# omid-arhami/topolow

Measured on AMD Instinct MI355X. Metric: relaxation iterations/sec (NxN pairs), higher is better.
Workload: dtype f32

## Files before the change

topolow_amd/csrc/relax_symm.h:

```cpp
#pragma once

#include <hip/hip_runtime.h>
#include <algorithm>
#include <type_traits>
#include <vector>
#include "relax_common.h"

namespace topolow {

#ifndef TOPOLOW_SYM_MINW
#define TOPOLOW_SYM_MINW 2
#endif
constexpr int kSymRows = 64;
constexpr int kSymCols = 32;
constexpr int kSymTileWords = kSymRows * kSymCols;
constexpr int kSymWaves = 4;

template <int DIM> struct SymRec { static constexpr int W = (DIM + 2 + 3) & ~3; };

struct SymUnit {
  int tile_row;
  int j0, j1;
  int tile0;
};

TL_HD inline long long sym_tile_index(int R, int J, int TC) { return (long long)R * TC - (long long)R * (R - 1) + (J - 2 * R); }
TL_HD inline size_t sym_word_in_tile(int r, int c) {
  const int a = r >> 3, p = (r & 7) >> 1, e = r & 1, b = c >> 2, h = (c & 3) >> 1, f = c & 1;
  return (size_t)((((4 * h + p) * 64) + a + 8 * b) * 4 + 2 * (f ^ (a & 1)) + e);
}

struct alignas(32) SymRun {
  int u0, u1;
  SymUnit first;
  int tiles;
  int reserved;
};
struct SymPlan {
  std::vector<SymUnit> units;
  std::vector<int> wave_first;
  std::vector<int2> row_units;
  std::vector<SymRun> runs() const {
    std::vector<SymRun> r(wave_first.size() - 1);
    for (size_t w = 0; w + 1 < wave_first.size(); ++w) {
      r[w].u0 = wave_first[w];
      r[w].u1 = wave_first[w + 1];
      r[w].first = r[w].u0 < r[w].u1 ? units[r[w].u0] : SymUnit{0, 0, 0, 0};
      r[w].tiles = 0;
      for (int u = r[w].u0; u < r[w].u1; ++u) r[w].tiles += units[u].j1 - units[u].j0;
      r[w].reserved = 0;
    }
    return r;
  }
};
inline SymPlan relax_symm_plan(int npad, int n_waves, long long t0 = 0, long long t1 = -1, int* r_first = nullptr,
                               int* r_last = nullptr) {
  SymPlan P;
  const int TR = npad / kSymRows, TC = npad / kSymCols;
  if (t1 < 0) t1 = (long long)TR * (TR + 1);
  const long long total = t1 - t0;
  int rf = -1, rl = -1;
  for (int R = 0; R < TR; ++R) {
    const long long a = sym_tile_index(R, 2 * R, TC), b = a + (TC - 2 * R);
// ... 63 lines not shown
  for (int R = 0; R < TR; ++R) {
    int j0 = 0, j1 = 0;
    rows_j(R, j0, j1);
    if (j1 > j0) total += j1 - j0;
  }
  P.wave_first.assign(n_waves + 1, 0);
  P.row_units.assign(TR, int2{0, 0});
  if (total == 0) return P;
  long long done = 0;
  int w = 0;
  long long w_end = (total * (w + 1) + n_waves - 1) / n_waves;
  for (int R = 0; R < TR; ++R) {
    P.row_units[R].x = (int)P.units.size();
    int j = 0, j_end = 0;
    rows_j(R, j, j_end);
    while (j < j_end) {
      while (done >= w_end && w + 1 < n_waves) {
        ++w;
        P.wave_first[w] = (int)P.units.size();
        w_end = (total * (w + 1) + n_waves - 1) / n_waves;
      }
      const int take = (int)std::min<long long>(j_end - j, std::max<long long>(w_end - done, 1));
      P.units.push_back({R, j, j + take, (int)sym_tile_index(R, j, TC)});
      j += take;
      done += take;
    }
    P.row_units[R].y = (int)P.units.size() - P.row_units[R].x;
  }
  for (int q = w + 1; q <= n_waves; ++q) P.wave_first[q] = (int)P.units.size();
  return P;
}

typedef float symf2 __attribute__((ext_vector_type(2)));
#ifdef TOPOLOW_SYM_STAMPS
__device__ unsigned long long* g_sym_stamps = nullptr;
#endif

#define TL_SYM_DPP_ADD(v, ctrl) asm volatile("v_add_f32_dpp %0, %0, %0 " ctrl " row_mask:0xf bank_mask:0xf" : "+v"(v))
template <int NV>
__device__ __forceinline__ void sym_col_reduce(float (&first)[NV], float (&second)[NV]) {
#pragma unroll
  for (int q = 0; q < NV; ++q) asm volatile("" : "+v"(first[q]), "+v"(second[q]));
  asm volatile("s_nop 1");
#pragma unroll
  for (int q = 0; q < NV; ++q)
    asm volatile("v_add_f32_dpp %0, %1, %0 quad_perm:[1,0,3,2] row_mask:0xf bank_mask:0xf" : "+v"(first[q]) : "v"(second[q]));
  if constexpr (NV < 3) asm volatile("s_nop 1");
#pragma unroll
  for (int q = 0; q < NV; ++q) TL_SYM_DPP_ADD(first[q], "quad_perm:[2,3,0,1]");
  if constexpr (NV < 3) asm volatile("s_nop 1");
#pragma unroll
  for (int q = 0; q < NV; ++q) TL_SYM_DPP_ADD(first[q], "row_shl:4");
}

template <int DIM, bool THR, bool ERR, bool CNT, bool FIRST>
__device__ __forceinline__ void sym_pair(const float (&pc)[DIM], float ksc, float cgc, const symf2 (&pi2)[DIM],
                                         symf2 ks2, symf2 cg2, uint32_t w0, uint32_t w1, symf2 (&racc2)[DIM],
                                         symf2 (&cacc2)[DIM], symf2& err2, unsigned& cnt_wave ) {
  symf2 dx[DIM];
  symf2 s = {0.0f, 0.0f};
#pragma unroll
  for (int d = 0; d < DIM; ++d) {
    const symf2 pcd = {pc[d], pc[d]};
    dx[d] = pcd - pi2[d];
    s = __builtin_elementwise_fma(dx[d], dx[d], s);
  }
  const symf2 r = {__builtin_amdgcn_sqrtf(s.x), __builtin_amdgcn_sqrtf(s.y)};
  const symf2 rs = r + (symf2){0.01f, 0.01f};
  const symf2 inv = {__builtin_amdgcn_rcpf(rs.x), __builtin_amdgcn_rcpf(rs.y)};
  const symf2 t = {bits_f32(THR ? (w0 & ~kCodeMask) : w0), bits_f32(THR ? (w1 & ~kCodeMask) : w1)};
  bool sp0, sp1;
  if constexpr (THR) {
    const symf2 e0 = t - r;
    auto decide = [](uint32_t w, float e) {
      const uint32_t flip = (w << 30) & 0x80000000u;
      const int32_t some = (int32_t)(((w >> 1) | w) << 31) >> 31;
      const uint32_t q = ((f32_bits(e) ^ flip) & (uint32_t)some) | (0x3f800000u & ~(uint32_t)some);
      return bits_f32(q) > 0.0f;
    };
    sp0 = decide(w0, e0.x);
    sp1 = decide(w1, e0.y);
  } else {
    sp0 = __builtin_amdgcn_classf(bits_f32(w0), 0x1f8);
    sp1 = __builtin_amdgcn_classf(bits_f32(w1), 0x1f8);
  }
  const symf2 e = t - r;
  const symf2 inv2 = inv * inv;
  const symf2 u = {sp0 ? e.x : inv2.x, sp1 ? e.y : inv2.y};
  const symf2 base = u * inv;
  const symf2 mr = {sp0 ? ks2.x : cg2.x, sp1 ? ks2.y : cg2.y};
  const symf2 coef = base * mr;
#pragma unroll
  for (int d = 0; d < DIM; ++d) racc2[d] = __builtin_elementwise_fma(dx[d], coef, racc2[d]);
  const symf2 mc = {sp0 ? ksc : cgc, sp1 ? ksc : cgc};
  const symf2 cc = base * mc;
#pragma unroll
  for (int d = 0; d < DIM; ++d)
    cacc2[d] = FIRST ? dx[d] * cc : __builtin_elementwise_fma(dx[d], cc, cacc2[d]);
  if constexpr (ERR) {
    const symf2 a = {sp0 ? fabsf(e.x) : 0.0f, sp1 ? fabsf(e.y) : 0.0f};
    err2 += a;
    if constexpr (CNT) cnt_wave += (sp0 ? 1u : 0u) + (sp1 ? 1u : 0u);
  }
}

template <int DIM, bool ANYTHR, bool ERR>
__global__ __launch_bounds__(64 * kSymWaves, TOPOLOW_SYM_MINW) void symm_sweep_kernel(
    const uint32_t* __restrict__ enc, const float* __restrict__ rec, const SymUnit* __restrict__ units,
    const SymRun* __restrict__ runs, float* __restrict__ rowpart, float* __restrict__ colpart, int npad,
    const RunState* st, double* __restrict__ part_sum, unsigned long long* __restrict__ part_cnt,
    unsigned long long fixed_cnt, int col_row0, int prio) {
  const int wave = __builtin_amdgcn_readfirstlane(threadIdx.x >> 6);
  const int gw = blockIdx.x * kSymWaves + wave;
  const SymRun run = runs[gw];
  int stopped = st->stopped;
  if constexpr (ERR)
    asm("" : "+s"(stopped) : "s"(run.u0), "s"(run.u1), "s"(run.first.tile_row), "s"(run.first.j0), "s"(run.first.j1),
        "s"(run.first.tile0), "s"(run.tiles), "s"(enc), "s"(rec), "s"(units),
        "s"(rowpart), "s"(colpart), "s"(npad), "s"(col_row0), "s"(prio), "s"(part_sum), "s"(part_cnt), "s"(fixed_cnt));
  else
    asm("" : "+s"(stopped) : "s"(run.u0), "s"(run.u1), "s"(run.first.tile_row), "s"(run.first.j0), "s"(run.first.j1),
        "s"(run.first.tile0), "s"(run.tiles), "s"(enc), "s"(rec), "s"(units),
        "s"(rowpart), "s"(colpart), "s"(npad), "s"(col_row0), "s"(prio));
  if (stopped) return;
#ifdef TOPOLOW_SYM_STAMPS
  const unsigned long long stamp_c0 = __builtin_amdgcn_s_memtime(), stamp_r0 = __builtin_amdgcn_s_memrealtime();
#endif
  constexpr int W = SymRec<DIM>::W;
  constexpr int kRecVec = W / 4;
  constexpr int kTileVec = kSymCols * kRecVec;
  constexpr int kLdsVec = kTileVec + kSymCols / 4;
  __shared__ uint4 lds[kSymWaves][2][kLdsVec];
  auto lds_slot = [](int q) { return q + (q / (4 * kRecVec)); };
  const int lane = threadIdx.x & 63;
  const int a = lane & 7, b = lane >> 3;

  const int u_begin = __builtin_amdgcn_readfirstlane(run.u0);
  const int u_end = __builtin_amdgcn_readfirstlane(run.u1);
  typedef unsigned int u32x4 __attribute__((ext_vector_type(4)));
  const __amdgpu_buffer_rsrc_t rec_rsrc = __builtin_amdgcn_make_buffer_rsrc(const_cast<float*>(rec), 0, npad * W * 4, 0x00020000);
  int left = __builtin_amdgcn_readfirstlane(run.tiles);
  const int lv3 = (3 * left) >> 2, lv2 = left >> 1, lv1 = left >> 2;
  SymUnit U_next = run.first;
  for (int u = u_begin; u < u_end; ++u) {
    const SymUnit U = U_next;
    U_next = units[u + 1 < u_end ? u + 1 : u];
    const int R = __builtin_amdgcn_readfirstlane(U.tile_row);
    const int J0 = __builtin_amdgcn_readfirstlane(U.j0), J1 = __builtin_amdgcn_readfirstlane(U.j1);
    __builtin_assume(J0 < J1);
    const int slot = u;
    const int tile0 = __builtin_amdgcn_readfirstlane(U.tile0);

    symf2 pi2[4][DIM], ks2[4], cg2[4], racc2[4][DIM];
    {
      const uint4* rr = reinterpret_cast<const uint4*>(rec + (size_t)(R * kSymRows + 8 * a) * W);
#pragma unroll
      for (int p = 0; p < 4; ++p) {
        float f[2][W];
#pragma unroll
        for (int e = 0; e < 2; ++e)
#pragma unroll
          for (int v = 0; v < kRecVec; ++v) {
            const uint4 q = rr[(2 * p + e) * kRecVec + v];
            f[e][4 * v + 0] = __builtin_bit_cast(float, q.x);
            f[e][4 * v + 1] = __builtin_bit_cast(float, q.y);
            f[e][4 * v + 2] = __builtin_bit_cast(float, q.z);
            f[e][4 * v + 3] = __builtin_bit_cast(float, q.w);
          }
#pragma unroll
        for (int d = 0; d < DIM; ++d) {
          pi2[p][d] = (symf2){f[0][d], f[1][d]};
          racc2[p][d] = (symf2){0.0f, 0.0f};
        }
        ks2[p] = (symf2){f[0][DIM], f[1][DIM]};
        cg2[p] = (symf2){f[0][DIM + 1], f[1][DIM + 1]};
      }
    }
    const __amdgpu_buffer_rsrc_t rsrc = __builtin_amdgcn_make_buffer_rsrc(
        const_cast<uint32_t*>(enc) + (size_t)tile0 * kSymTileWords, 0, (J1 - J0) * kSymTileWords * 4, 0x00020000);
    const __amdgpu_buffer_rsrc_t col_rsrc = __builtin_amdgcn_make_buffer_rsrc(colpart + (size_t)(R - col_row0) * npad * DIM, 0, npad * DIM * 4, 0x00020000);
    const int col_off = a < 2 ? (4 * b + a) * DIM * 4 : 0x40000000;
    const int swap = a & 1;
    auto request = [&](int J, int h, u32x4 (&dst)[4]) {
#pragma unroll
      for (int p = 0; p < 4; ++p)
        dst[p] = __builtin_amdgcn_raw_buffer_load_b128(rsrc, lane * 16 + ((J - J0) * 8 + 4 * h + p) * 1024, 0, 0);
    };
    u32x4 wa[4], wb[4];
    request(J0, 0, wa);
    const uint4* recv = reinterpret_cast<const uint4*>(rec);
    if (lane < kTileVec) lds[wave][J0 & 1][lds_slot(lane)] = recv[(size_t)J0 * kTileVec + lane];
    if constexpr (kTileVec > 64) if (lane + 64 < kTileVec) lds[wave][J0 & 1][lds_slot(lane + 64)] = recv[(size_t)J0 * kTileVec + lane + 64];

    symf2 err2 = {0.0f, 0.0f};
    float err_unit = 0.0f;
    unsigned cnt_wave = 0, cnt_unit2 = 0;
    auto read_rec = [&](int J, int idx, float (&f)[W]) {
      const int col = idx ^ swap;
      const uint4* cp = &lds[wave][J & 1][4 * b * kRecVec + b];
#pragma unroll
      for (int v = 0; v < kRecVec; ++v) {
        const uint4 q = cp[col * kRecVec + v];
        f[4 * v + 0] = __builtin_bit_cast(float, q.x);
        f[4 * v + 1] = __builtin_bit_cast(float, q.y);
        f[4 * v + 2] = __builtin_bit_cast(float, q.z);
        f[4 * v + 3] = __builtin_bit_cast(float, q.w);
      }
    };
    float f_first[W];
    read_rec(J0, 0, f_first);
#pragma unroll 1
    for (int J = J0; J < J1; ++J) {
      if (prio) {
        if (left > lv3) __builtin_amdgcn_s_setprio(3);
        else if (left > lv2) __builtin_amdgcn_s_setprio(2);
        else if (left > lv1) __builtin_amdgcn_s_setprio(1);
        else __builtin_amdgcn_s_setprio(0);
      }
      --left;
      const int Jn = J + 1 < J1 ? J + 1 : J;
      request(J, 1, wb);
      u32x4 rn0 = {0, 0, 0, 0}, rn1 = {0, 0, 0, 0};
      rn0 = __builtin_amdgcn_raw_buffer_load_b128(rec_rsrc, (Jn * kTileVec + lane) * 16, 0, 0);
      if constexpr (kTileVec > 64) rn1 = __builtin_amdgcn_raw_buffer_load_b128(rec_rsrc, (Jn * kTileVec + lane + 64) * 16, 0, 0);
      __builtin_amdgcn_sched_barrier(0);

      const bool diag = J < 2 * R + 2;
      float fq[4][W];
#pragma unroll
      for (int q = 0; q < W; ++q) fq[0][q] = f_first[q];
      auto half = [&](auto hc, const u32x4 (&wc)[4]) {
        constexpr int h = decltype(hc)::value;
        symf2 cacc2[2][DIM];
#pragma unroll
        for (int c = 0; c < 2; ++c) {
          if (2 * h + c + 1 < 4) {
            read_rec(J, 2 * h + c + 1, fq[2 * h + c + 1]);
            __builtin_amdgcn_sched_barrier(0);
          }
          const float (&f)[W] = fq[2 * h + c];
          float pc[DIM];
#pragma unroll
          for (int d = 0; d < DIM; ++d) pc[d] = f[d];
          const float ksc = f[DIM], cgc = f[DIM + 1];
#pragma unroll
          for (int p = 0; p < 4; ++p) {
            const uint32_t w0 = c == 0 ? wc[p].x : wc[p].z, w1 = c == 0 ? wc[p].y : wc[p].w;
            if (p == 0)
              sym_pair<DIM, ANYTHR, ERR, ANYTHR, true>(pc, ksc, cgc, pi2[p], ks2[p], cg2[p], w0, w1, racc2[p], cacc2[c], err2, cnt_wave);
            else
              sym_pair<DIM, ANYTHR, ERR, ANYTHR, false>(pc, ksc, cgc, pi2[p], ks2[p], cg2[p], w0, w1, racc2[p], cacc2[c], err2, cnt_wave);
          }
        }
        float first[DIM], second[DIM];
#pragma unroll
        for (int d = 0; d < DIM; ++d) {
          first[d] = cacc2[0][d].x + cacc2[0][d].y;
          second[d] = cacc2[1][d].x + cacc2[1][d].y;
        }
        sym_col_reduce<DIM>(first, second);
        const int off0 = col_off + ((J * kSymCols) * DIM + h * 2 * DIM) * 4;
#pragma unroll
        for (int q = 0; q < DIM; q += 4) {
          if (q + 4 <= DIM) {
            const u32x4 pk = {__builtin_bit_cast(uint32_t, first[q]), __builtin_bit_cast(uint32_t, first[q + 1]),
                              __builtin_bit_cast(uint32_t, first[q + 2]), __builtin_bit_cast(uint32_t, first[q + 3])};
            __builtin_amdgcn_raw_buffer_store_b128(pk, col_rsrc, off0 + q * 4, 0, 0);
          } else {
#pragma unroll
            for (int t = q; t < DIM; ++t)
              __builtin_amdgcn_raw_buffer_store_b32(__builtin_bit_cast(uint32_t, first[t]), col_rsrc, off0 + t * 4, 0, 0);
          }
        }
      };
      half(std::integral_constant<int, 0>{}, wa);
      request(Jn, 0, wa);
      __builtin_amdgcn_sched_barrier(0);
      half(std::integral_constant<int, 1>{}, wb);
      if constexpr (ERR) {
        const float es = err2.x + err2.y;
        err_unit += diag ? es : 2.0f * es;
        cnt_unit2 += diag ? cnt_wave : 2u * cnt_wave;
        err2 = (symf2){0.0f, 0.0f};
        cnt_wave = 0;
      }
      __builtin_amdgcn_sched_barrier(0);
      if (lane < kTileVec) lds[wave][(J + 1) & 1][lds_slot(lane)] = make_uint4(rn0.x, rn0.y, rn0.z, rn0.w);
      if constexpr (kTileVec > 64) if (lane + 64 < kTileVec) lds[wave][(J + 1) & 1][lds_slot(lane + 64)] = make_uint4(rn1.x, rn1.y, rn1.z, rn1.w);
      read_rec(J + 1, 0, f_first);
    }
#pragma unroll
    for (int p = 0; p < 4; ++p)
#pragma unroll
      for (int d = 0; d < DIM; ++d) {
        symf2 v = racc2[p][d];
        v.x += __shfl_xor(v.x, 8, 64);  v.y += __shfl_xor(v.y, 8, 64);
        v.x += __shfl_xor(v.x, 16, 64); v.y += __shfl_xor(v.y, 16, 64);
        v.x += __shfl_xor(v.x, 32, 64); v.y += __shfl_xor(v.y, 32, 64);
        racc2[p][d] = v;
      }
    if (b == 0) {
      float* dst = rowpart + ((size_t)slot * kSymRows + 8 * a) * DIM;
#pragma unroll
      for (int p = 0; p < 4; ++p)
#pragma unroll
        for (int d = 0; d < DIM; ++d) {
          dst[(2 * p) * DIM + d] = racc2[p][d].x;
          dst[(2 * p + 1) * DIM + d] = racc2[p][d].y;
        }
    }
    if constexpr (ERR) {
      double s = (double)err_unit;
#pragma unroll
      for (int m = 32; m >= 1; m >>= 1) s += __shfl_xor(s, m, 64);
      if constexpr (ANYTHR) {
#pragma unroll
        for (int m = 32; m >= 1; m >>= 1) cnt_unit2 += __shfl_xor(cnt_unit2, m, 64);
      }
      if (lane == 0) {
        part_sum[slot] = s;
        part_cnt[slot] = ANYTHR ? (unsigned long long)cnt_unit2 : (slot == 0 ? fixed_cnt : 0ull);
      }
    }
  }
#ifdef TOPOLOW_SYM_STAMPS
  if (lane == 0 && g_sym_stamps != nullptr) {
    g_sym_stamps[4 * gw] = __builtin_amdgcn_s_memtime() - stamp_c0;
    g_sym_stamps[4 * gw + 1] = stamp_r0;
    g_sym_stamps[4 * gw + 2] = __builtin_amdgcn_s_memrealtime();
    unsigned hw_id, xcc_id;
    asm volatile("s_getreg_b32 %0, hwreg(HW_REG_HW_ID)" : "=s"(hw_id));
    asm volatile("s_getreg_b32 %0, hwreg(HW_REG_XCC_ID)" : "=s"(xcc_id));
    g_sym_stamps[4 * gw + 3] = ((unsigned long long)xcc_id << 32) | hw_id;
  }
#endif
}

template <int DIM, typename real> struct SymReal;
template <int DIM> struct SymReal<DIM, float> {
  static constexpr int W = SymRec<DIM>::W;
  __device__ static float ks(double k, float g) { return (float)(2.0 * k) / (4.0f * g + (float)k); }
  __device__ static float cg(double c_rep, float g) { return (float)(0.5 * c_rep) / g; }
  __device__ static float far(int) { return kFarF32; }
};

#ifndef TL_APPLY_PARTS
#define TL_APPLY_PARTS 16
#endif
constexpr int kSymApplyParts = TL_APPLY_PARTS;
template <int DIM, typename real>
__global__ __launch_bounds__(32 * kSymApplyParts) void symm_apply_kernel(
    const real* __restrict__ rec, real* __restrict__ rec_next, real* __restrict__ pos_out, const float* __restrict__ gplus,
    const real* __restrict__ rowpart, const real* __restrict__ colpart, const int2* __restrict__ row_units, int n,
    int npad, double k_next, double c_rep, int iter1, RunState* st, int rr_stages = 0, int rr_stage = 0) {
// ... 81 lines not shown
}

__global__ __launch_bounds__(256) void symm_tiles_kernel(const uint32_t* const* __restrict__ src, const int* __restrict__ row0,
                                                        int n_src, int ld, uint32_t* __restrict__ tenc, int TC,
                                                        long long t_first) {
  const long long t = t_first + blockIdx.x;
  int R = 0;
  {
    const double b = (double)TC + 1.0;
    const double disc = b * b - 4.0 * (double)t;
    R = (int)((b - sqrt(disc > 0.0 ? disc : 0.0)) * 0.5);
    while (R > 0 && (long long)R * TC - (long long)R * (R - 1) > t) --R;
    while ((long long)(R + 1) * TC - (long long)(R + 1) * R <= t) ++R;
  }
  const int J = 2 * R + (int)(t - ((long long)R * TC - (long long)R * (R - 1)));
  uint32_t* dst = tenc + (size_t)blockIdx.x * kSymTileWords;
  const int rows = row0[n_src];
#pragma unroll
  for (int q = 0; q < kSymTileWords / 256; ++q) {
    const int cell = threadIdx.x + q * 256;
    const int r = cell >> 5, c = cell & 31;
    const int row = R * kSymRows + r, col = J * kSymCols + c;
    uint32_t w = kInfWord;
    if (row < rows && col < ld) {
      int blk = 0;
      while (blk + 1 < n_src && row >= row0[blk + 1]) ++blk;
      w = src[blk][enc_index(row - row0[blk], col, ld)];
    }
    const int a = r >> 3, p = (r & 7) >> 1, e = r & 1, b = c >> 2, h = (c & 3) >> 1, f = c & 1;
    dst[(((4 * h + p) * 64) + a + 8 * b) * 4 + 2 * (f ^ (a & 1)) + e] = w;
  }
}


template <int DIM>
__global__ __launch_bounds__(32 * 32) void symm_partial_kernel(
    const float* __restrict__ rowpart, const float* __restrict__ colpart, const int2* __restrict__ row_units, int r_first,
    int r_last, int n, int npad, float* const* __restrict__ inbox, const int* __restrict__ own0, int n_own, int slot,
    const RunState* st) {
  if (st != nullptr && st->stopped) return;
  __shared__ float red[32][kSymCols][DIM];
  const int R = blockIdx.x >> 1;
  const int part = threadIdx.x >> 5, pt = threadIdx.x & 31;
  const int i = blockIdx.x * kSymCols + pt;
  float acc[DIM];
#pragma unroll
  for (int d = 0; d < DIM; ++d) acc[d] = 0.0f;
  const int r_stop = R < r_last + 1 ? R : r_last + 1;
  for (int Rp = r_first + part; Rp < r_stop; Rp += 32) {
    const float* src = colpart + ((size_t)(Rp - r_first) * npad + i) * DIM;
#pragma unroll
    for (int d = 0; d < DIM; ++d) acc[d] += src[d];
  }
  if (R >= r_first && R <= r_last) {
    const int2 ru = row_units[R - r_first];
    const int row_in_tile = i - R * kSymRows;
    for (int q = part; q < ru.y; q += 32) {
      const float* src = rowpart + ((size_t)(ru.x + q) * kSymRows + row_in_tile) * DIM;
#pragma unroll
      for (int d = 0; d < DIM; ++d) acc[d] -= src[d];
    }
  }
#pragma unroll
  for (int d = 0; d < DIM; ++d) red[part][pt][d] = acc[d];
  __syncthreads();
  if (part == 0 && i < n) {
// ... 40 lines not shown
```

topolow_amd/csrc/topolow_relax.hip:

```cpp

#include <hip/hip_runtime.h>

#include <chrono>
#include <cstdarg>
#include <cstdio>
#include <algorithm>
#include <cstring>
#include <cstdlib>
#include <array>
#include <atomic>
#include <deque>
#include <mutex>
#include <string>
#include <memory>
#include <thread>
#include <vector>

#include "../../include/topolow_relax.h"
#include "relax_common.h"
#include "relax_host.h"
#include "relax_kernels.h"
#include "relax_fold.h"
#include "relax_gs.h"
#include "relax_tilegs.h"
// ... 117 lines not shown
  DevBuf<double> part_sum;
  DevBuf<unsigned long long> part_cnt;
  DevBuf<RunState> state;
  RunState* mailbox = nullptr;
  RunState* mailbox_dev = nullptr;
  double* trace = nullptr;
  double* trace_dev = nullptr;
  int trace_cap = 0;

  int n_iter = 0, check_freq = 3, window = 5, fixed_stages = 0;
  double k0 = 0, cooling = 0, c_rep = 0, eps = 1e-4;
  uint64_t seed = 0;
  int iters_enqueued = 0;
  double k_host = 0;
  int cur = 0;
  bool host_seen_stop = false;
  bool began = false;
  long long stage_launches = 0;
  std::deque<hipEvent_t> pending;
  std::vector<hipEvent_t> event_pool;
  DevBuf<void*> push_tab[3];
  int n_push = 0;
  DevBuf<double> rank_sum;
  DevBuf<unsigned long long> rank_cnt;
  DevBuf<double*> rsum_tab;
  DevBuf<unsigned long long*> rcnt_tab;
  int n_ranks = 0, rank = 0;
  struct SymState {
    bool allowed = false;
    int min_n = 0;
    bool ready = false;
    int npad = 0, tiles = 0, grid = 0;
    DevBuf<uint32_t> tenc;
    DevBuf<unsigned char> rec[2], rowpart, colpart;
    int rec_cur = 0, rec_iter = -1;
    DevBuf<float> tdelta;
    bool delta_ready = false;
    struct Plan {
      DevBuf<SymUnit> units;
      DevBuf<SymRun> runs;
      DevBuf<int2> row_units;
      int n_units = 0;
      void load(const SymPlan& hp) {
        const std::vector<SymRun> hr = hp.runs();
        n_units = (int)hp.units.size();
        units.alloc(std::max<size_t>(hp.units.size(), 1));
        runs.alloc(hr.size());
        row_units.alloc(std::max<size_t>(hp.row_units.size(), 1));
        if (!hp.units.empty())
          HIP_TRY(hipMemcpy(units.p, hp.units.data(), hp.units.size() * sizeof(SymUnit), hipMemcpyHostToDevice));
        HIP_TRY(hipMemcpy(runs.p, hr.data(), hr.size() * sizeof(SymRun), hipMemcpyHostToDevice));
        if (!hp.row_units.empty())
          HIP_TRY(hipMemcpy(row_units.p, hp.row_units.data(), hp.row_units.size() * sizeof(int2), hipMemcpyHostToDevice));
      }
      void release() { units.release(); runs.release(); row_units.release(); n_units = 0; }
    };
    Plan plan;
    std::vector<Plan> rr[4];
    bool whole = false;
    bool two_stage = true;
    bool prio = true;
    int rr_min_tiles = 5;
    DevBuf<const uint32_t*> src_tab;
    DevBuf<int> src_row0;
    bool seg_ready = false;
    bool seg_thr = false;
    int seg_first = 0, seg_last = -1;
    int seg_slots = 0;
    int seg_slot = 0;
    bool seg_caller = false;
    DevBuf<float> inbox;
    DevBuf<float*> inbox_tab;
    DevBuf<int> own0;
    std::vector<const void*> seg_peers;

    void release() {
      tenc.release(); rec[0].release(); rec[1].release(); rowpart.release(); colpart.release();
      tdelta.release(); delta_ready = false;
      plan.release();
      for (auto& v : rr) v.clear();
      src_tab.release(); src_row0.release();
      inbox.release(); inbox_tab.release(); own0.release();
    }
  } sym;
  int fused_parts = 0;
  bool profiling = false;
  std::vector<std::pair<hipEvent_t, hipEvent_t>> prof_stage, prof_stage_err, prof_check;
  std::vector<std::pair<hipEvent_t, hipEvent_t>> prof_sym, prof_sym_err;

  size_t real_size() const { return precision == TOPOLOW_PRECISION_F64 ? 8 : 4; }
  int rows() const { return row_end - row_begin; }
  int pos_rows() const { return (n + 3) & ~3; }

  ~topolow_session() {
    for (auto& pr : prof_stage) { (void)hipEventDestroy(pr.first); (void)hipEventDestroy(pr.second); }
    for (auto& pr : prof_stage_err) { (void)hipEventDestroy(pr.first); (void)hipEventDestroy(pr.second); }
    for (auto& pr : prof_check) { (void)hipEventDestroy(pr.first); (void)hipEventDestroy(pr.second); }
    for (auto& pr : prof_sym) { (void)hipEventDestroy(pr.first); (void)hipEventDestroy(pr.second); }
    for (auto& pr : prof_sym_err) { (void)hipEventDestroy(pr.first); (void)hipEventDestroy(pr.second); }
    for (hipEvent_t e : pending) (void)hipEventDestroy(e);
    for (hipEvent_t e : event_pool) (void)hipEventDestroy(e);
    if (mailbox) (void)hipHostFree(mailbox);
    if (trace) (void)hipHostFree(trace);
    if (ev_iter_done) (void)hipEventDestroy(ev_iter_done);
    if (ev_check_done) (void)hipEventDestroy(ev_check_done);
    if (check_stream) (void)hipStreamDestroy(check_stream);
    if (own_stream) (void)hipStreamDestroy(own_stream);
  }
};

// ... 411 lines not shown
               long long t0, long long t1) {
  auto& y = s->sym;
  y.npad = (s->n + kSymRows - 1) & ~(kSymRows - 1);
  const int TR = y.npad / kSymRows, TC = y.npad / kSymCols;
  if (t1 < 0) t1 = (long long)TR * (TR + 1);
  y.tiles = (int)(t1 - t0);
  hipDeviceProp_t prop;
  HIP_TRY(hipGetDeviceProperties(&prop, s->device));
  int occ = 1 << 30;
  auto probe = [&](auto kern) {
    int per_cu = 0;
    HIP_TRY(hipOccupancyMaxActiveBlocksPerMultiprocessor(&per_cu, kern, 64 * kSymWaves, 0));
    occ = std::min(occ, std::max(1, per_cu));
  };
  const bool f64 = s->precision == TOPOLOW_PRECISION_F64;
  sym_real(s, [&](auto r) {
    sym_sweep_instance<DIM, decltype(r)>(any_thr, false, probe);
    sym_sweep_instance<DIM, decltype(r)>(any_thr, true, probe);
  });
  y.grid = occ * prop.multiProcessorCount;
  y.plan.load(relax_symm_plan(y.npad, y.grid * kSymWaves, t0, t1, &y.seg_first, &y.seg_last));
  y.whole = t0 == 0 && (long long)y.tiles == (long long)TR * (TR + 1);
  for (auto& v : y.rr) v.clear();
  const int max_units = std::max(y.plan.n_units, y.grid * kSymWaves + 2 * TR + 8);
  y.src_tab.alloc(src.size());
  y.src_row0.alloc(row0.size());
  HIP_TRY(hipMemcpy(y.src_tab.p, src.data(), src.size() * sizeof(const uint32_t*), hipMemcpyHostToDevice));
  HIP_TRY(hipMemcpy(y.src_row0.p, row0.data(), row0.size() * sizeof(int), hipMemcpyHostToDevice));
  y.tenc.alloc((size_t)std::max(y.tiles, 1) * kSymTileWords);
  if (y.tiles > 0)
    hipLaunchKernelGGL(symm_tiles_kernel, dim3(y.tiles), dim3(256), 0, s->stream, y.src_tab.p, y.src_row0.p, (int)src.size(),
                       s->ld, y.tenc.p, TC, t0);
  HIP_TRY(hipGetLastError());
  const int seg_rows = y.seg_last >= y.seg_first ? y.seg_last - y.seg_first + 1 : 1;
  const size_t rs = s->real_size();
  for (auto& r : y.rec) r.alloc((size_t)y.npad * (f64 ? SymRec64<DIM>::W : SymRec<DIM>::W) * rs);
  y.rowpart.alloc((size_t)std::max(max_units, 1) * kSymRows * DIM * rs);
  y.colpart.alloc((size_t)seg_rows * y.npad * DIM * rs);
  HIP_TRY(hipMemsetAsync(y.colpart.p, 0, (size_t)seg_rows * y.npad * DIM * rs, s->stream));
  if (f64) {
    y.delta_ready = false;
    if (s->list_is_block && !s->dense_mae && s->n_edges > 0 && y.whole) {
      y.tdelta.alloc((size_t)y.tiles * kSymTileWords);
      HIP_TRY(hipMemsetAsync(y.tdelta.p, 0, (size_t)y.tiles * kSymTileWords * sizeof(float), s->stream));
      hipLaunchKernelGGL(symm64_delta_kernel, dim3(2048), dim3(256), 0, s->stream, s->ei.p, s->ej.p, (const double*)s->et.p,
                         s->ec.p, (long long)s->n_edges, y.tdelta.p, TC, s->n);
      HIP_TRY(hipGetLastError());
      y.delta_ready = true;
    }
  }
  if ((size_t)y.plan.n_units > s->part_sum.n) {
    HIP_TRY(hipStreamSynchronize(s->stream));
    HIP_TRY(hipStreamSynchronize(s->check_stream));
    s->part_sum.alloc(y.plan.n_units);
    s->part_cnt.alloc(y.plan.n_units);
  }
  y.rec_iter = -1;
}

template <int DIM>
void sym_prepare(topolow_session* s) {
  sym_build<DIM>(s, {s->enc.p}, {0, s->rows()}, s->any_threshold, 0, -1);
  s->sym.ready = true;
  s->sym.seg_ready = false;
}

// ... 1 lines not shown
  if (s->sym.ready) return true;
  try {
    TL_DISPATCH_SYM(s->dim, sym_prepare, s);
  } catch (const HipError&) {
    (void)hipGetLastError();
    s->sym.release();
    s->sym.ready = false;
    s->sym.allowed = false;
  }
  return s->sym.ready;
}

template <int DIM>
void sym_records(topolow_session* s, const void* pin, void* rec, double k) {
  sym_real(s, [&](auto r) {
    using real = decltype(r);
    hipLaunchKernelGGL((symm_records_kernel<DIM, real>), dim3((s->sym.npad + 255) / 256), dim3(256), 0, s->stream,
                       (const real*)pin, s->gplus.p, (real*)rec, s->n, s->sym.npad, k, s->c_rep);
  });
}

template <int DIM>
void sym_sweep(topolow_session* s, const SymPlanDev& plan, const void* rec, bool thr, bool err,
               unsigned long long block_cells, int col_row0, bool prio) {
  auto& y = s->sym;
  sym_real(s, [&](auto r) {
    using real = decltype(r);
    sym_sweep_instance<DIM, real>(thr, err, [&](auto kern) {
      if constexpr (std::is_same<real, double>::value)
        hipLaunchKernelGGL(kern, dim3(y.grid), dim3(64 * kSymWaves), 0, s->stream, y.tenc.p, (const double*)rec,
                           plan.units.p, plan.runs.p, (double*)y.rowpart.p, (double*)y.colpart.p, y.npad, s->state.p,
                           col_row0, y.tdelta.p, s->part_sum.p, s->part_cnt.p, block_cells);
      else
        hipLaunchKernelGGL(kern, dim3(y.grid), dim3(64 * kSymWaves), 0, s->stream, y.tenc.p, (const float*)rec,
                           plan.units.p, plan.runs.p, (float*)y.rowpart.p, (float*)y.colpart.p, y.npad, s->state.p,
                           s->part_sum.p, s->part_cnt.p, block_cells, col_row0, prio && y.prio ? 1 : 0);
    });
  });
}

template <int DIM>
void sym_apply(topolow_session* s, const SymPlanDev& plan, const void* rec, void* rec_next, void* pout, double k_next,
               int iter, int rr_stages, int rr_stage) {
  auto& y = s->sym;
  sym_real(s, [&](auto r) {
    using real = decltype(r);
    hipLaunchKernelGGL((symm_apply_kernel<DIM, real>), dim3(y.npad / kSymCols), dim3(32 * kSymApplyParts), 0, s->stream,
                       (const real*)rec, (real*)rec_next, (real*)pout, s->gplus.p, (const real*)y.rowpart.p,
                       (const real*)y.colpart.p, plan.row_units.p, s->n, y.npad, k_next, s->c_rep, iter + 1, s->state.p,
                       rr_stages, rr_stage);
  });
}

bool sym_rr_stages_ok(int S) { return S == 2 || S == 4 || S == 8; }
int sym_rr_log2(int S) { return S == 2 ? 1 : (S == 4 ? 2 : 3); }

bool sym_rr_available(topolow_session* s, int S) {
  auto& y = s->sym;
  if (!sym_rr_stages_ok(S) || !y.whole) return false;
  const int TR = y.npad / kSymRows;
  if (TR < 2 * S) return false;
  if ((long long)TR * (TR + 1) / S < (long long)y.rr_min_tiles * y.grid * kSymWaves) return false;
  const int lg = sym_rr_log2(S);
  if (!y.rr[lg].empty()) return true;
  std::vector<SymPlanDev> plans(S);
  for (int st = 0; st < S; ++st) {
    const SymPlan hp = relax_symm_plan_rows(y.npad, y.grid * kSymWaves, [&](int R, int& j0, int& j1) { sym_rr_row(TR, S, st, R, j0, j1); });
// ... 1746 lines not shown
```

Before: 17970.

## Precompute per-tile spring masks and prefetch next unit's head loads across units

Adds a setup kernel that precomputes, per tile, 64-bit wave ballot masks marking which pairs are springs. In the non-threshold sweep these are loaded as scalars and expanded with inverse_ballot, replacing the per-pair float class test. The next unit's row records, first tile words and column records are now prefetched before the current unit's reductions, and row records are staged through LDS. The row and error reductions now use permlane swaps and DPP in place of shuffle_xor, and part_cnt initialisation is hoisted. This adds scalar mask loads, more LDS and register pressure, and a one-time mask kernel.

```diff
diff --git a/topolow_amd/csrc/relax_symm.h b/topolow_amd/csrc/relax_symm.h
--- a/topolow_amd/csrc/relax_symm.h
+++ b/topolow_amd/csrc/relax_symm.h
@@ -5,15 +5,13 @@
 #include <type_traits>
 #include <vector>
 #include "relax_common.h"
+#include "relax_symm_layout.h"
 
 namespace topolow {
 
 #ifndef TOPOLOW_SYM_MINW
 #define TOPOLOW_SYM_MINW 2
 #endif
-constexpr int kSymRows = 64;
-constexpr int kSymCols = 32;
-constexpr int kSymTileWords = kSymRows * kSymCols;
 constexpr int kSymWaves = 4;
 
 template <int DIM> struct SymRec { static constexpr int W = (DIM + 2 + 3) & ~3; };
@@ -25,10 +23,6 @@
 };
 
 TL_HD inline long long sym_tile_index(int R, int J, int TC) { return (long long)R * TC - (long long)R * (R - 1) + (J - 2 * R); }
-TL_HD inline size_t sym_word_in_tile(int r, int c) {
-  const int a = r >> 3, p = (r & 7) >> 1, e = r & 1, b = c >> 2, h = (c & 3) >> 1, f = c & 1;
-  return (size_t)((((4 * h + p) * 64) + a + 8 * b) * 4 + 2 * (f ^ (a & 1)) + e);
-}
 
 struct alignas(32) SymRun {
   int u0, u1;
@@ -158,6 +152,7 @@
 }
 
 typedef float symf2 __attribute__((ext_vector_type(2)));
+typedef uint32_t symu16 __attribute__((ext_vector_type(16)));
 #ifdef TOPOLOW_SYM_STAMPS
 __device__ unsigned long long* g_sym_stamps = nullptr;
 #endif
@@ -179,9 +174,73 @@
   for (int q = 0; q < NV; ++q) TL_SYM_DPP_ADD(first[q], "row_shl:4");
 }
 
+typedef uint32_t symu2 __attribute__((ext_vector_type(2)));
+template <int CTRL>
+__device__ __forceinline__ uint32_t sym_dpp(uint32_t x) { return (uint32_t)__builtin_amdgcn_mov_dpp((int)x, CTRL, 0xf, 0xf, false); }
+constexpr int kDppRor8 = 0x128, kDppXor2 = 0x4e, kDppXor1 = 0xb1, kDppShl4 = 0x104, kDppShr4 = 0x114;
+__device__ __forceinline__ uint32_t sym_dpp_xor4(uint32_t x) {
+  const int t = __builtin_amdgcn_update_dpp(0, (int)x, kDppShl4, 0xf, 0x5, false);
+  return (uint32_t)__builtin_amdgcn_update_dpp(t, (int)x, kDppShr4, 0xf, 0xa, false);
+}
+__device__ __forceinline__ double sym_wave_sum(double s) {
+  auto dbl = [](uint32_t lo, uint32_t hi) { return __builtin_bit_cast(double, ((uint64_t)hi << 32) | lo); };
+  auto lo_of = [](double v) { return (uint32_t)__builtin_bit_cast(uint64_t, v); };
+  auto hi_of = [](double v) { return (uint32_t)(__builtin_bit_cast(uint64_t, v) >> 32); };
+  {
+    const symu2 l = __builtin_amdgcn_permlane32_swap(lo_of(s), lo_of(s), false, false);
+    const symu2 h = __builtin_amdgcn_permlane32_swap(hi_of(s), hi_of(s), false, false);
+    s = dbl(l[0], h[0]) + dbl(l[1], h[1]);
+  }
+  {
+    const symu2 l = __builtin_amdgcn_permlane16_swap(lo_of(s), lo_of(s), false, false);
+    const symu2 h = __builtin_amdgcn_permlane16_swap(hi_of(s), hi_of(s), false, false);
+    s = dbl(l[0], h[0]) + dbl(l[1], h[1]);
+  }
+  s += dbl(sym_dpp<kDppRor8>(lo_of(s)), sym_dpp<kDppRor8>(hi_of(s)));
+  s += dbl(sym_dpp_xor4(lo_of(s)), sym_dpp_xor4(hi_of(s)));
+  s += dbl(sym_dpp<kDppXor2>(lo_of(s)), sym_dpp<kDppXor2>(hi_of(s)));
+  s += dbl(sym_dpp<kDppXor1>(lo_of(s)), sym_dpp<kDppXor1>(hi_of(s)));
+  return s;
+}
+__device__ __forceinline__ unsigned sym_wave_sum(unsigned s) {
+  symu2 r = __builtin_amdgcn_permlane32_swap(s, s, false, false);
+  s = r[0] + r[1];
+  r = __builtin_amdgcn_permlane16_swap(s, s, false, false);
+  s = r[0] + r[1];
+  s += sym_dpp<kDppRor8>(s);
+  s += sym_dpp_xor4(s);
+  s += sym_dpp<kDppXor2>(s);
+  s += sym_dpp<kDppXor1>(s);
+  return s;
+}
+template <int DIM>
+__device__ __forceinline__ void sym_row_reduce(const symf2 (&racc2)[4][DIM], float (&out)[2 * DIM]) {
+  constexpr int G = 2 * DIM;
+  float v[8 * DIM];
+#pragma unroll
+  for (int p = 0; p < 4; ++p)
+#pragma unroll
+    for (int d = 0; d < DIM; ++d) {
+      const symf2 own = racc2[p][d];
+      const symf2 oth = {bits_f32(sym_dpp<kDppRor8>(f32_bits(own.x))), bits_f32(sym_dpp<kDppRor8>(f32_bits(own.y)))};
+      const symf2 sum = own + oth;
+      v[(2 * p) * DIM + d] = sum.x;
+      v[(2 * p + 1) * DIM + d] = sum.y;
+    }
+#pragma unroll
+  for (int g = 0; g < G; ++g) {
+    const symu2 xy = __builtin_amdgcn_permlane16_swap(f32_bits(v[g]), f32_bits(v[g + G]), false, false);
+    const symu2 zw = __builtin_amdgcn_permlane16_swap(f32_bits(v[g + 2 * G]), f32_bits(v[g + 3 * G]), false, false);
+    const float s = bits_f32(xy[0]) + bits_f32(xy[1]), t = bits_f32(zw[0]) + bits_f32(zw[1]);
+    const symu2 st = __builtin_amdgcn_permlane32_swap(f32_bits(s), f32_bits(t), false, false);
+    out[g] = bits_f32(st[0]) + bits_f32(st[1]);
+  }
+}
+
 template <int DIM, bool THR, bool ERR, bool CNT, bool FIRST>
 __device__ __forceinline__ void sym_pair(const float (&pc)[DIM], float ksc, float cgc, const symf2 (&pi2)[DIM],
-                                         symf2 ks2, symf2 cg2, uint32_t w0, uint32_t w1, symf2 (&racc2)[DIM],
+                                         symf2 ks2, symf2 cg2, uint32_t w0, uint32_t w1, uint64_t m0, uint64_t m1, symf2 eps,
+                                         symf2 (&racc2)[DIM],
                                          symf2 (&cacc2)[DIM], symf2& err2, unsigned& cnt_wave ) {
   symf2 dx[DIM];
   symf2 s = {0.0f, 0.0f};
@@ -192,7 +251,7 @@
     s = __builtin_elementwise_fma(dx[d], dx[d], s);
   }
   const symf2 r = {__builtin_amdgcn_sqrtf(s.x), __builtin_amdgcn_sqrtf(s.y)};
-  const symf2 rs = r + (symf2){0.01f, 0.01f};
+  const symf2 rs = r + eps;
   const symf2 inv = {__builtin_amdgcn_rcpf(rs.x), __builtin_amdgcn_rcpf(rs.y)};
   const symf2 t = {bits_f32(THR ? (w0 & ~kCodeMask) : w0), bits_f32(THR ? (w1 & ~kCodeMask) : w1)};
   bool sp0, sp1;
@@ -207,8 +266,8 @@
     sp0 = decide(w0, e0.x);
     sp1 = decide(w1, e0.y);
   } else {
-    sp0 = __builtin_amdgcn_classf(bits_f32(w0), 0x1f8);
-    sp1 = __builtin_amdgcn_classf(bits_f32(w1), 0x1f8);
+    sp0 = __builtin_amdgcn_inverse_ballot_w64(m0);
+    sp1 = __builtin_amdgcn_inverse_ballot_w64(m1);
   }
   const symf2 e = t - r;
   const symf2 inv2 = inv * inv;
@@ -232,8 +291,8 @@
 
 template <int DIM, bool ANYTHR, bool ERR>
 __global__ __launch_bounds__(64 * kSymWaves, TOPOLOW_SYM_MINW) void symm_sweep_kernel(
-    const uint32_t* __restrict__ enc, const float* __restrict__ rec, const SymUnit* __restrict__ units,
-    const SymRun* __restrict__ runs, float* __restrict__ rowpart, float* __restrict__ colpart, int npad,
+    const uint32_t* __restrict__ enc, const unsigned long long* __restrict__ masks, const float* __restrict__ rec,
+    const SymUnit* __restrict__ units, const SymRun* __restrict__ runs, float* __restrict__ rowpart, float* __restrict__ colpart, int npad,
     const RunState* st, double* __restrict__ part_sum, unsigned long long* __restrict__ part_cnt,
     unsigned long long fixed_cnt, int col_row0, int prio) {
   const int wave = __builtin_amdgcn_readfirstlane(threadIdx.x >> 6);
@@ -242,11 +301,11 @@
   int stopped = st->stopped;
   if constexpr (ERR)
     asm("" : "+s"(stopped) : "s"(run.u0), "s"(run.u1), "s"(run.first.tile_row), "s"(run.first.j0), "s"(run.first.j1),
-        "s"(run.first.tile0), "s"(run.tiles), "s"(enc), "s"(rec), "s"(units),
+        "s"(run.first.tile0), "s"(run.tiles), "s"(enc), "s"(masks), "s"(rec), "s"(units),
         "s"(rowpart), "s"(colpart), "s"(npad), "s"(col_row0), "s"(prio), "s"(part_sum), "s"(part_cnt), "s"(fixed_cnt));
   else
     asm("" : "+s"(stopped) : "s"(run.u0), "s"(run.u1), "s"(run.first.tile_row), "s"(run.first.j0), "s"(run.first.j1),
-        "s"(run.first.tile0), "s"(run.tiles), "s"(enc), "s"(rec), "s"(units),
+        "s"(run.first.tile0), "s"(run.tiles), "s"(enc), "s"(masks), "s"(rec), "s"(units),
         "s"(rowpart), "s"(colpart), "s"(npad), "s"(col_row0), "s"(prio));
   if (stopped) return;
 #ifdef TOPOLOW_SYM_STAMPS
@@ -255,19 +314,53 @@
   constexpr int W = SymRec<DIM>::W;
   constexpr int kRecVec = W / 4;
   constexpr int kTileVec = kSymCols * kRecVec;
-  constexpr int kLdsVec = kTileVec + kSymCols / 4;
+  constexpr int kLdsLanes = kTileVec < 64 ? 64 : kTileVec;
+  constexpr int kLdsVec = kLdsLanes + kLdsLanes / (4 * kRecVec);
   __shared__ uint4 lds[kSymWaves][2][kLdsVec];
   auto lds_slot = [](int q) { return q + (q / (4 * kRecVec)); };
+  constexpr int kRowVec = kSymRows * kRecVec;
+  __shared__ uint4 lds_row[kSymWaves][kRowVec + kSymRows / 8];
+  auto row_slot = [](int q) { return q + (q / (8 * kRecVec)); };
   const int lane = threadIdx.x & 63;
   const int a = lane & 7, b = lane >> 3;
+  symf2 eps = {0.01f, 0.01f};
+  asm volatile("" : "+v"(eps));
 
   const int u_begin = __builtin_amdgcn_readfirstlane(run.u0);
   const int u_end = __builtin_amdgcn_readfirstlane(run.u1);
+  if constexpr (ERR && !ANYTHR) {
+    for (int us = u_begin + lane; us < u_end; us += 64) part_cnt[us] = us == 0 ? fixed_cnt : 0ull;
+  }
   typedef unsigned int u32x4 __attribute__((ext_vector_type(4)));
-  const __amdgpu_buffer_rsrc_t rec_rsrc = __builtin_amdgcn_make_buffer_rsrc(const_cast<float*>(rec), 0, npad * W * 4, 0x00020000);
-  int left = __builtin_amdgcn_readfirstlane(run.tiles);
-  const int lv3 = (3 * left) >> 2, lv2 = left >> 1, lv1 = left >> 2;
+  auto rec_buffer = [&]() {
+    const float* r = rec;
+    asm volatile("" : "+s"(r));
+    return __builtin_amdgcn_make_buffer_rsrc(const_cast<float*>(r), 0, npad * W * 4, 0x00020000);
+  };
+  const int run_tiles = __builtin_amdgcn_readfirstlane(run.tiles);
+  float* const col_base = colpart - (ptrdiff_t)col_row0 * npad * DIM;
+  int left = prio ? run_tiles : -1;
+  __amdgpu_buffer_rsrc_t rsrc;
+  u32x4 wa[4], wb[4], rq[kRecVec], rh0 = {0, 0, 0, 0}, rh1 = {0, 0, 0, 0};
+  symu16 mk_first = {};
+  auto request_head = [&](const SymUnit& V) {
+    const int Rv = __builtin_amdgcn_readfirstlane(V.tile_row), Jv0 = __builtin_amdgcn_readfirstlane(V.j0);
+    const int Jv1 = __builtin_amdgcn_readfirstlane(V.j1), tv0 = __builtin_amdgcn_readfirstlane(V.tile0);
+    const __amdgpu_buffer_rsrc_t rec_rsrc = rec_buffer();
+#pragma unroll
+    for (int v = 0; v < kRecVec; ++v)
+      rq[v] = __builtin_amdgcn_raw_buffer_load_b128(rec_rsrc, (Rv * kRowVec + lane + 64 * v) * 16, 0, 0);
+    rsrc = __builtin_amdgcn_make_buffer_rsrc(const_cast<uint32_t*>(enc) + (ptrdiff_t)(tv0 - Jv0) * kSymTileWords, 0,
+                                             Jv1 * kSymTileWords * 4, 0x00020000);
+#pragma unroll
+    for (int p = 0; p < 4; ++p) wa[p] = __builtin_amdgcn_raw_buffer_load_b128(rsrc, lane * 16 + p * 1024, Jv0 * 8192, 0);
+    rh0 = __builtin_amdgcn_raw_buffer_load_b128(rec_rsrc, (Jv0 * kTileVec + lane) * 16, 0, 0);
+    if constexpr (kTileVec > 64) rh1 = __builtin_amdgcn_raw_buffer_load_b128(rec_rsrc, (Jv0 * kTileVec + lane + 64) * 16, 0, 0);
+    if constexpr (!ANYTHR)
+      mk_first = *reinterpret_cast<const symu16*>(reinterpret_cast<const char*>(masks) + (uint32_t)tv0 * (kSymTileMasks * 8u));
+  };
   SymUnit U_next = run.first;
+  request_head(U_next);
   for (int u = u_begin; u < u_end; ++u) {
     const SymUnit U = U_next;
     U_next = units[u + 1 < u_end ? u + 1 : u];
@@ -275,11 +368,14 @@
     const int J0 = __builtin_amdgcn_readfirstlane(U.j0), J1 = __builtin_amdgcn_readfirstlane(U.j1);
     __builtin_assume(J0 < J1);
     const int slot = u;
-    const int tile0 = __builtin_amdgcn_readfirstlane(U.tile0);
+    const int j_diag_end = 2 * R + 2;
+    const int tile_less_j = __builtin_amdgcn_readfirstlane(U.tile0) - J0;
 
     symf2 pi2[4][DIM], ks2[4], cg2[4], racc2[4][DIM];
     {
-      const uint4* rr = reinterpret_cast<const uint4*>(rec + (size_t)(R * kSymRows + 8 * a) * W);
+#pragma unroll
+      for (int v = 0; v < kRecVec; ++v) lds_row[wave][row_slot(lane + 64 * v)] = make_uint4(rq[v].x, rq[v].y, rq[v].z, rq[v].w);
+      const uint4* rr = &lds_row[wave][8 * a * kRecVec + a];
 #pragma unroll
       for (int p = 0; p < 4; ++p) {
         float f[2][W];
@@ -302,21 +398,16 @@
         cg2[p] = (symf2){f[0][DIM + 1], f[1][DIM + 1]};
       }
     }
-    const __amdgpu_buffer_rsrc_t rsrc = __builtin_amdgcn_make_buffer_rsrc(
-        const_cast<uint32_t*>(enc) + (size_t)tile0 * kSymTileWords, 0, (J1 - J0) * kSymTileWords * 4, 0x00020000);
-    const __amdgpu_buffer_rsrc_t col_rsrc = __builtin_amdgcn_make_buffer_rsrc(colpart + (size_t)(R - col_row0) * npad * DIM, 0, npad * DIM * 4, 0x00020000);
+    const __amdgpu_buffer_rsrc_t col_rsrc = __builtin_amdgcn_make_buffer_rsrc(col_base + (size_t)R * npad * DIM, 0, npad * DIM * 4, 0x00020000);
     const int col_off = a < 2 ? (4 * b + a) * DIM * 4 : 0x40000000;
     const int swap = a & 1;
     auto request = [&](int J, int h, u32x4 (&dst)[4]) {
 #pragma unroll
       for (int p = 0; p < 4; ++p)
-        dst[p] = __builtin_amdgcn_raw_buffer_load_b128(rsrc, lane * 16 + ((J - J0) * 8 + 4 * h + p) * 1024, 0, 0);
+        dst[p] = __builtin_amdgcn_raw_buffer_load_b128(rsrc, lane * 16 + p * 1024, (J * 2 + h) * 4096, 0);
     };
-    u32x4 wa[4], wb[4];
-    request(J0, 0, wa);
-    const uint4* recv = reinterpret_cast<const uint4*>(rec);
-    if (lane < kTileVec) lds[wave][J0 & 1][lds_slot(lane)] = recv[(size_t)J0 * kTileVec + lane];
-    if constexpr (kTileVec > 64) if (lane + 64 < kTileVec) lds[wave][J0 & 1][lds_slot(lane + 64)] = recv[(size_t)J0 * kTileVec + lane + 64];
+    lds[wave][J0 & 1][lds_slot(lane)] = make_uint4(rh0.x, rh0.y, rh0.z, rh0.w);
+    if constexpr (kTileVec > 64) if (lane + 64 < kTileVec) lds[wave][J0 & 1][lds_slot(lane + 64)] = make_uint4(rh1.x, rh1.y, rh1.z, rh1.w);
 
     symf2 err2 = {0.0f, 0.0f};
     float err_unit = 0.0f;
@@ -333,35 +424,52 @@
         f[4 * v + 3] = __builtin_bit_cast(float, q.w);
       }
     };
+    auto read_masks = [&](int J, int idx) -> symu16 {
+      if constexpr (ANYTHR) return symu16{};
+      else return *reinterpret_cast<const symu16*>(reinterpret_cast<const char*>(masks) +
+                                                   ((uint32_t)(J + tile_less_j) * (kSymTileMasks * 8u) + idx * 64u));
+    };
     float f_first[W];
     read_rec(J0, 0, f_first);
+    asm volatile("" : : "s"(U_next.tile_row), "s"(U_next.j0), "s"(U_next.j1), "s"(U_next.tile0));
 #pragma unroll 1
     for (int J = J0; J < J1; ++J) {
-      if (prio) {
-        if (left > lv3) __builtin_amdgcn_s_setprio(3);
-        else if (left > lv2) __builtin_amdgcn_s_setprio(2);
-        else if (left > lv1) __builtin_amdgcn_s_setprio(1);
-        else __builtin_amdgcn_s_setprio(0);
-      }
+      if (4 * left > 3 * run_tiles) __builtin_amdgcn_s_setprio(3);
+      else if (2 * left > run_tiles) __builtin_amdgcn_s_setprio(2);
+      else if (4 * left > run_tiles) __builtin_amdgcn_s_setprio(1);
+      else __builtin_amdgcn_s_setprio(0);
       --left;
       const int Jn = J + 1 < J1 ? J + 1 : J;
       request(J, 1, wb);
       u32x4 rn0 = {0, 0, 0, 0}, rn1 = {0, 0, 0, 0};
+      const __amdgpu_buffer_rsrc_t rec_rsrc = rec_buffer();
       rn0 = __builtin_amdgcn_raw_buffer_load_b128(rec_rsrc, (Jn * kTileVec + lane) * 16, 0, 0);
       if constexpr (kTileVec > 64) rn1 = __builtin_amdgcn_raw_buffer_load_b128(rec_rsrc, (Jn * kTileVec + lane + 64) * 16, 0, 0);
       __builtin_amdgcn_sched_barrier(0);
 
-      const bool diag = J < 2 * R + 2;
+      const bool diag = J < j_diag_end;
       float fq[4][W];
+      symu16 mk[4];
 #pragma unroll
       for (int q = 0; q < W; ++q) fq[0][q] = f_first[q];
+      mk[0] = mk_first;
       auto half = [&](auto hc, const u32x4 (&wc)[4]) {
         constexpr int h = decltype(hc)::value;
         symf2 cacc2[2][DIM];
 #pragma unroll
         for (int c = 0; c < 2; ++c) {
           if (2 * h + c + 1 < 4) {
+            if constexpr (!ANYTHR) {
+              if (c > 0) __builtin_amdgcn_sched_barrier(0);
+              asm volatile("" : : "v"(fq[2 * h + c][W - 1]), "s"(mk[2 * h + c]));
+            }
             read_rec(J, 2 * h + c + 1, fq[2 * h + c + 1]);
+            mk[2 * h + c + 1] = read_masks(J, 2 * h + c + 1);
+            __builtin_amdgcn_sched_barrier(0);
+          } else if constexpr (!ANYTHR) {
+            __builtin_amdgcn_sched_barrier(0);
+            asm volatile("" : : "v"(fq[2 * h + c][W - 1]), "s"(mk[2 * h + c]));
+            mk_first = read_masks(Jn, 0);
             __builtin_amdgcn_sched_barrier(0);
           }
           const float (&f)[W] = fq[2 * h + c];
@@ -372,10 +480,12 @@
 #pragma unroll
           for (int p = 0; p < 4; ++p) {
             const uint32_t w0 = c == 0 ? wc[p].x : wc[p].z, w1 = c == 0 ? wc[p].y : wc[p].w;
+            const symu16& mq = mk[2 * h + c];
+            const uint64_t m0 = ((uint64_t)mq[4 * p + 1] << 32) | mq[4 * p], m1 = ((uint64_t)mq[4 * p + 3] << 32) | mq[4 * p + 2];
             if (p == 0)
-              sym_pair<DIM, ANYTHR, ERR, ANYTHR, true>(pc, ksc, cgc, pi2[p], ks2[p], cg2[p], w0, w1, racc2[p], cacc2[c], err2, cnt_wave);
+              sym_pair<DIM, ANYTHR, ERR, ANYTHR, true>(pc, ksc, cgc, pi2[p], ks2[p], cg2[p], w0, w1, m0, m1, eps, racc2[p], cacc2[c], err2, cnt_wave);
             else
-              sym_pair<DIM, ANYTHR, ERR, ANYTHR, false>(pc, ksc, cgc, pi2[p], ks2[p], cg2[p], w0, w1, racc2[p], cacc2[c], err2, cnt_wave);
+              sym_pair<DIM, ANYTHR, ERR, ANYTHR, false>(pc, ksc, cgc, pi2[p], ks2[p], cg2[p], w0, w1, m0, m1, eps, racc2[p], cacc2[c], err2, cnt_wave);
           }
         }
         float first[DIM], second[DIM];
@@ -411,41 +521,38 @@
         cnt_wave = 0;
       }
       __builtin_amdgcn_sched_barrier(0);
-      if (lane < kTileVec) lds[wave][(J + 1) & 1][lds_slot(lane)] = make_uint4(rn0.x, rn0.y, rn0.z, rn0.w);
+      lds[wave][(J + 1) & 1][lds_slot(lane)] = make_uint4(rn0.x, rn0.y, rn0.z, rn0.w);
       if constexpr (kTileVec > 64) if (lane + 64 < kTileVec) lds[wave][(J + 1) & 1][lds_slot(lane + 64)] = make_uint4(rn1.x, rn1.y, rn1.z, rn1.w);
       read_rec(J + 1, 0, f_first);
     }
-#pragma unroll
-    for (int p = 0; p < 4; ++p)
-#pragma unroll
-      for (int d = 0; d < DIM; ++d) {
-        symf2 v = racc2[p][d];
-        v.x += __shfl_xor(v.x, 8, 64);  v.y += __shfl_xor(v.y, 8, 64);
-        v.x += __shfl_xor(v.x, 16, 64); v.y += __shfl_xor(v.y, 16, 64);
-        v.x += __shfl_xor(v.x, 32, 64); v.y += __shfl_xor(v.y, 32, 64);
-        racc2[p][d] = v;
+    if (u + 1 < u_end) {
+      request_head(U_next);
+    } else {
+#pragma unroll
+      for (int v = 0; v < kRecVec; ++v) asm volatile("" : "=v"(rq[v]));
+      asm volatile("" : "=v"(rh0));
+      asm volatile("" : "=v"(rh1));
+    }
+    __builtin_amdgcn_sched_barrier(0);
+    {
+      float tot[2 * DIM];
+      sym_row_reduce<DIM>(racc2, tot);
+      int lane_end = lane;
+      asm volatile("" : "+v"(lane_end));
+      if ((lane_end & 8) == 0) {
+        float* dst = rowpart + ((size_t)slot * kSymRows + 8 * a) * DIM + (b >> 1) * 2 * DIM;
+#pragma unroll
+        for (int g = 0; g < 2 * DIM; ++g) dst[g] = tot[g];
       }
-    if (b == 0) {
-      float* dst = rowpart + ((size_t)slot * kSymRows + 8 * a) * DIM;
-#pragma unroll
-      for (int p = 0; p < 4; ++p)
-#pragma unroll
-        for (int d = 0; d < DIM; ++d) {
-          dst[(2 * p) * DIM + d] = racc2[p][d].x;
-          dst[(2 * p + 1) * DIM + d] = racc2[p][d].y;
-        }
     }
     if constexpr (ERR) {
-      double s = (double)err_unit;
-#pragma unroll
-      for (int m = 32; m >= 1; m >>= 1) s += __shfl_xor(s, m, 64);
-      if constexpr (ANYTHR) {
-#pragma unroll
-        for (int m = 32; m >= 1; m >>= 1) cnt_unit2 += __shfl_xor(cnt_unit2, m, 64);
-      }
-      if (lane == 0) {
+      const double s = sym_wave_sum((double)err_unit);
+      if constexpr (ANYTHR) cnt_unit2 = sym_wave_sum(cnt_unit2);
+      int lane_err = lane;
+      asm volatile("" : "+v"(lane_err));
+      if (lane_err == 0) {
         part_sum[slot] = s;
-        part_cnt[slot] = ANYTHR ? (unsigned long long)cnt_unit2 : (slot == 0 ? fixed_cnt : 0ull);
+        if constexpr (ANYTHR) part_cnt[slot] = (unsigned long long)cnt_unit2;
       }
     }
   }
@@ -593,6 +700,25 @@
   }
 }
 
+__global__ __launch_bounds__(64) void symm_masks_kernel(const uint32_t* __restrict__ tenc, unsigned long long* __restrict__ masks) {
+  const int lane = threadIdx.x;
+  const uint4* tile = reinterpret_cast<const uint4*>(tenc + (size_t)blockIdx.x * kSymTileWords);
+  unsigned long long mine = 0;
+#pragma unroll
+  for (int h = 0; h < 2; ++h)
+#pragma unroll
+    for (int p = 0; p < 4; ++p) {
+      const uint4 q = tile[(4 * h + p) * 64 + lane];
+      const uint32_t w[4] = {q.x, q.y, q.z, q.w};
+#pragma unroll
+      for (int ce = 0; ce < 4; ++ce) {
+        const unsigned long long m = __ballot(__builtin_amdgcn_classf(bits_f32(w[ce]), 0x1f8));
+        if (lane == ((2 * h + (ce >> 1)) * 4 + p) * 2 + (ce & 1)) mine = m;
+      }
+    }
+  if (lane < kSymTileMasks) masks[(size_t)blockIdx.x * kSymTileMasks + lane] = mine;
+}
+
 
 template <int DIM>
 __global__ __launch_bounds__(32 * 32) void symm_partial_kernel(
diff --git a/topolow_amd/csrc/relax_symm_layout.h b/topolow_amd/csrc/relax_symm_layout.h
--- /dev/null
+++ b/topolow_amd/csrc/relax_symm_layout.h
@@ -0,0 +1,34 @@
+#pragma once
+
+#include <cstddef>
+#include <cstdint>
+
+#ifndef TL_HD
+#define TL_HD
+#endif
+
+namespace topolow {
+
+constexpr int kSymRows = 64;
+constexpr int kSymCols = 32;
+constexpr int kSymTileWords = kSymRows * kSymCols;
+constexpr int kSymTileMasks = 32;
+
+TL_HD inline size_t sym_word_in_tile(int r, int c) {
+  const int a = r >> 3, p = (r & 7) >> 1, e = r & 1, b = c >> 2, h = (c & 3) >> 1, f = c & 1;
+  return (size_t)((((4 * h + p) * 64) + a + 8 * b) * 4 + 2 * (f ^ (a & 1)) + e);
+}
+
+inline void sym_tile_masks_host(const uint32_t* tile, unsigned long long* masks) {
+  for (int m = 0; m < kSymTileMasks; ++m) {
+    const int e = m & 1, p = (m >> 1) & 3, c = (m >> 3) & 1, h = m >> 4;
+    unsigned long long bits = 0;
+    for (int lane = 0; lane < 64; ++lane) {
+      const uint32_t w = tile[((4 * h + p) * 64 + lane) * 4 + 2 * c + e];
+      if ((w & 0x7f800000u) != 0x7f800000u) bits |= 1ull << lane;
+    }
+    masks[m] = bits;
+  }
+}
+
+}
diff --git a/topolow_amd/csrc/topolow_relax.hip b/topolow_amd/csrc/topolow_relax.hip
--- a/topolow_amd/csrc/topolow_relax.hip
+++ b/topolow_amd/csrc/topolow_relax.hip
@@ -173,6 +173,7 @@
     bool ready = false;
     int npad = 0, tiles = 0, grid = 0;
     DevBuf<uint32_t> tenc;
+    DevBuf<unsigned long long> tmask;
     DevBuf<unsigned char> rec[2], rowpart, colpart;
     int rec_cur = 0, rec_iter = -1;
     DevBuf<float> tdelta;
@@ -216,7 +217,7 @@
     std::vector<const void*> seg_peers;
 
     void release() {
-      tenc.release(); rec[0].release(); rec[1].release(); rowpart.release(); colpart.release();
+      tenc.release(); tmask.release(); rec[0].release(); rec[1].release(); rowpart.release(); colpart.release();
       tdelta.release(); delta_ready = false;
       plan.release();
       for (auto& v : rr) v.clear();
@@ -694,6 +695,11 @@
     hipLaunchKernelGGL(symm_tiles_kernel, dim3(y.tiles), dim3(256), 0, s->stream, y.src_tab.p, y.src_row0.p, (int)src.size(),
                        s->ld, y.tenc.p, TC, t0);
   HIP_TRY(hipGetLastError());
+  if (!f64) {
+    y.tmask.alloc((size_t)std::max(y.tiles, 1) * kSymTileMasks);
+    if (y.tiles > 0) hipLaunchKernelGGL(symm_masks_kernel, dim3(y.tiles), dim3(64), 0, s->stream, y.tenc.p, y.tmask.p);
+    HIP_TRY(hipGetLastError());
+  }
   const int seg_rows = y.seg_last >= y.seg_first ? y.seg_last - y.seg_first + 1 : 1;
   const size_t rs = s->real_size();
   for (auto& r : y.rec) r.alloc((size_t)y.npad * (f64 ? SymRec64<DIM>::W : SymRec<DIM>::W) * rs);
@@ -761,7 +767,7 @@
                            plan.units.p, plan.runs.p, (double*)y.rowpart.p, (double*)y.colpart.p, y.npad, s->state.p,
                            col_row0, y.tdelta.p, s->part_sum.p, s->part_cnt.p, block_cells);
       else
-        hipLaunchKernelGGL(kern, dim3(y.grid), dim3(64 * kSymWaves), 0, s->stream, y.tenc.p, (const float*)rec,
+        hipLaunchKernelGGL(kern, dim3(y.grid), dim3(64 * kSymWaves), 0, s->stream, y.tenc.p, y.tmask.p, (const float*)rec,
                            plan.units.p, plan.runs.p, (float*)y.rowpart.p, (float*)y.colpart.p, y.npad, s->state.p,
                            s->part_sum.p, s->part_cnt.p, block_cells, col_row0, prio && y.prio ? 1 : 0);
     });
```

New measurement: 19030, median of 6. 1.06x the previous value.
